# ecmwf-ifs/ecwam

Hardware: AMD Instinct MI355X
Metric: grid-point spectral steps/sec (whole node) at O320, 36dir x 36freq (higher is better)
Workload: dtype f32; 1 GPU; O320 all-ocean octahedral grid, 421080 sea points, 36 dir x 36 freq (NFRE_RED=36), full WAMINTGR step = PROPAGS2 advection + NEWWIND + IMPLSCH as one kernel (PROPAGS2 inside IMPLSCH's tile load), IDELT=IDELPRO=450 s, flag set A (IPHYS=1, ISNONLIN=0, LLGCBZ0=F, LLNORMAGAM=F); points_per_gpu=421080, halo_points=0, parallelism=sea-point block x1, ranks=1

## Files before the change

### ecwam_amd/build.py

```python
from __future__ import annotations

import hashlib
import os
import re
import shutil
import subprocess
import sys

HERE = os.path.dirname(os.path.abspath(__file__))
CSRC = os.path.join(HERE, "csrc")
LIBDIR = os.path.join(HERE, "lib")
LIB = os.path.join(LIBDIR, "libecwam_hip.so")
SOURCES = ["capi.hip", "propag.hip", "implsch4.hip", "implsch4a.hip", "implsch4x.hip", "implsch4r.hip", "implsch4rd.hip", "outbs.hip", "outbs_sep.hip", "outbs_ext.hip"]
DERIVED = {"implsch4r.hip": ("implsch4r.hip", ["-DV4R_PREC=1"]), "implsch4rd.hip": ("implsch4r.hip", ["-DV4R_PREC=2", "-DV4R_DP=2"])}
HIPCC = shutil.which("hipcc") or "/opt/rocm/bin/hipcc"
FAST_DIV = ["-fno-hip-fp32-correctly-rounded-divide-sqrt"]
FLAGS = ["--offload-arch=gfx950", "-O3", "-fPIC", "-std=c++17", "-Wall", "-Wno-unused-variable", "-Wno-unused-but-set-variable"]
IMPLSCH_SOURCES = ("implsch4.hip", "implsch4a.hip", "implsch4x.hip", "implsch4r.hip", "implsch4rd.hip")
VARIANTS = {"": FAST_DIV, "exactdiv": ["-DECWAM_HIP_STRICT=0"], "strict1": ["-DECWAM_HIP_STRICT=1"], "strict2": FAST_DIV + ["-DECWAM_HIP_STRICT=2"],
            "site4": ["-DECWAM_HIP_STRICT=4"], "site8": ["-DECWAM_HIP_STRICT=8"], "site32": ["-DECWAM_HIP_STRICT=32"],
            "strict3": ["-DECWAM_HIP_STRICT=3"], "strict7": ["-DECWAM_HIP_STRICT=3", "-ffp-contract=off"],
            "noieee": FAST_DIV + ["-mno-amdgpu-ieee", "-fno-honor-nans"],
            "rdp": FAST_DIV + ["-O3", "-DV4R_DP=1"], "rdpchk": FAST_DIV + ["-O3", "-DV4R_DP=1", "-DV4_CHECK=1"], "rdpO2": FAST_DIV + ["-O2", "-DV4R_DP=1"],
            "split": FAST_DIV + ["-DV4_SPLIT_ALL=1", "-DV4R_DP=2"],
            "norecpf": FAST_DIV + ["-DV4_RECPF=0"], "norecs": FAST_DIV + ["-DV4_RECV=0"], "noredn": FAST_DIV + ["-DV4_REDN=0"],
            "advprobe": FAST_DIV + ["-DV4_ADV_PROBE=1"],
            "ctustrict": FAST_DIV,
            "advO1": FAST_DIV + ["-O1"],
            "advd2": FAST_DIV + ["-DV4_ADV_DEPTH=2"], "advd4": FAST_DIV + ["-DV4_ADV_DEPTH=4"], "advprio": FAST_DIV + ["-DV4_ADV_PRIO=2"]}
VARIANT_ANY = {"ctustrict": ["-DECWAM_HIP_CTU_STRICT=1"]}
VARIANT_SOURCES = {"ctustrict": ("propag.hip", "implsch4a.hip"), "advprobe": ("implsch4a.hip",), "advO1": ("implsch4a.hip",), "advd2": ("implsch4a.hip",), "advd4": ("implsch4a.hip",),
                   "advprio": ("implsch4a.hip",), "rdp": ("implsch4rd.hip",), "rdpchk": ("implsch4rd.hip",), "rdpO2": ("implsch4rd.hip",),
                   "split": ("implsch4.hip", "implsch4x.hip", "implsch4r.hip", "implsch4rd.hip"), "norecpf": ("implsch4.hip",), "norecs": ("implsch4.hip",),
                   "noredn": ("implsch4.hip",)}

INCLUDE = os.path.join(HERE, "..", "include", "ecwam_hip.h")


def lib_path(variant: str = "") -> str:
    return LIB if not variant else os.path.join(LIBDIR, f"libecwam_hip_{variant}.so")


def _closure(path: str, seen: dict) -> None:
    path = os.path.normpath(path)
    if path in seen or not os.path.exists(path):
        return
    with open(path, "rb") as fh:
        data = fh.read()
    seen[path] = data
    for m in re.finditer(rb'^[ \t]*#[ \t]*include[ \t]*"([^"]+)"', data, re.M):
        _closure(os.path.join(os.path.dirname(path), m.group(1).decode()), seen)


def _stamp(src: str, flags: list) -> str:
    seen: dict = {}
    _closure(os.path.join(CSRC, src), seen)
    h = hashlib.sha256(" ".join([HIPCC, *flags]).encode())
    for k in sorted(seen):
        h.update(os.path.relpath(k, HERE).encode())
        h.update(seen[k])
    return h.hexdigest()


def build(force: bool = False, verbose: bool = False, variant: str = "") -> str:
    if variant not in VARIANTS:
# ... 90 lines not shown
```

### ecwam_amd/csrc/capi.hip

```cpp
#include <cmath>
#include <cstdio>
#include <cstdlib>
#include <cstring>
#include <string>
#include <vector>

#include <dlfcn.h>
#include <rccl/rccl.h>

#include "dev.h"
#include "implsch_adv_args.h"

static thread_local std::string g_err;
static int fail(const std::string& m) {
  g_err = m;
  return 1;
}
#define HIPCHK(x)                                                                        \
  do {                                                                                   \
    hipError_t e_ = (x);                                                                 \
    if (e_ != hipSuccess) return fail(std::string(#x) + ": " + hipGetErrorString(e_));   \
  } while (0)

struct ecwam_hip_ctx {
// ... 736 lines not shown
  if (!c) return fail("null context");
  if (!fused_ok(c) || !implsch4_adv_forms(c->NANG, c->real_bytes)) return fail("ecwam_hip_propags2_implsch: no one-kernel build covers the configuration (ecwam_hip_propags2_implsch_supported): call ecwam_hip_propags2_otf and ecwam_hip_implsch");
  if (kijl < kijs || kijs < 0 || kijl > n || nd3s < 1 || nd3e > c->NFRE_RED || nd3e < nd3s - 1) return fail("ecwam_hip_propags2_implsch: bad range");
  if (kijl > kijs && (!f1 || !f3 || !kxlt || !zdello || !cosph || !sinph || !klon || !klat || !kcor || !wlat || !wcor || !cgroup_ext || !cosphm1_ext ||
                      !wvprpt || !ff || !intf || !mij || !xllws))
    return fail("ecwam_hip_propags2_implsch: null pointer");
  if (f1 == f3) return fail("ecwam_hip_propags2_implsch: F1 and F3 must not alias (the neighbours of a point are read while other points are stored)");
  if (((uintptr_t)f1 % 16) != 0 || ((uintptr_t)f3 % 16) != 0) return fail("ecwam_hip_propags2_implsch: the spectra must be 16-byte aligned");
  if (ifrelfmax < 0 || ifrelfmax > c->NFRE_RED || (ifrelfmax > 0) != (gin != nullptr))
    return fail("ecwam_hip_propags2_implsch: fast waves (ifrelfmax > 0) come with their compact input rows (gin), and only then");
  if (gin && (nd3s != 1 || gin_nfre < ifrelfmax || gin_nfre > c->NFRE || gin_nfre % (16 / c->real_bytes) != 0 || ((uintptr_t)gin % 16) != 0 || gin == c->fast_g ||
              !(delpro_lf > 0.0)))
    return fail("ecwam_hip_propags2_implsch: the compact fast-wave rows must be 16-byte aligned, hold the fast waves in a multiple of 16 bytes per direction, and differ from the rows of ecwam_hip_set_fastwave_copy");
  if (c->p.lwnemocou && kijl > kijs && !wam2nemo) return fail("ecwam_hip_propags2_implsch: LWNEMOCOU needs the WAVE2OCEAN buffer");
  if (c->obs && kijl > c->n_obs) return fail("ecwam_hip_propags2_implsch: more points than the obstruction table holds");
  if (!c->p.lwnemocou) wam2nemo = nullptr;
  HIPCHK(hipSetDevice(c->device));
  hipStream_t s = (hipStream_t)stream;
  if (kijl == kijs) return 0;
  if (int rc2 = implsch_reserve_on(c, kijl, s, false)) return rc2;
  const size_t dir_reals = (size_t)(6 * c->NANG + 4);
  int* dirI = reinterpret_cast<int*>(reinterpret_cast<char*>(c->adv_dir) + dir_reals * c->real_bytes);
  const double dlf = gin ? delpro_lf : 0.0;
  DISPATCH(launch_ctu_prep<float>(c->dtab, kijs, kijl, ngy, delpro, dlf, kxlt, zdello, xdella, cosph, sinph, wlat, wcor, cosphm1_ext, c->adv_pt, c->adv_dir, dirI, s),
           launch_ctu_prep<double>(c->dtab, kijs, kijl, ngy, delpro, dlf, kxlt, zdello, xdella, cosph, sinph, wlat, wcor, cosphm1_ext, c->adv_pt, c->adv_dir, dirI, s));
  Implsch4AdvArgs a;
  a.f_in = f1; a.klon = klon; a.klat = klat; a.kcor = kcor; a.cg = cgroup_ext; a.pt = c->adv_pt; a.dirT = c->adv_dir; a.dirI = dirI;
  a.xdella = xdella; a.delpro = delpro; a.m0 = nd3s - 1; a.m1 = nd3e;
  a.gin = gin; a.delpro_lf = dlf; a.gin_k = gin ? gin_nfre : 0; a.mlf = gin ? ifrelfmax : 0;
  a.obs = c->obs;
  a.gfast = c->fast_g; a.gfast_k = c->fast_g ? c->fast_gk : 0;
  a.xcd_walk = (flags & 1) ? 1 : (((flags >> 8) & 0xFFF) > 1 ? ((flags >> 8) & 0xFFF) : 0);
  a.mode = (flags & 2) ? 2 : 1;
  const int ext = (c->p.llnormagam || c->p.llgcbz0) ? 1 : 0;
  int rc = -1;
  DISPATCH(rc = launch_implsch4_adv<float>(c->dtab, kijs, kijl, f3, wvprpt, ff, intf, mij, xllws, c->fin, wam2nemo, &a, c->NANG, c->NFRE, c->v4_r1, c->v4_r2, c->v4_nh, ext, s),
           rc = launch_implsch4_adv<double>(c->dtab, kijs, kijl, f3, wvprpt, ff, intf, mij, xllws, c->fin, wam2nemo, &a, c->NANG, c->NFRE, c->v4_r1, c->v4_r2, c->v4_nh, ext, s));
  if (rc != 0) return fail("ecwam_hip_propags2_implsch: no one-kernel build covers the configuration (the strict build of the weights has neither the fast-wave nor the obstruction form)");
  HIPCHK(hipGetLastError());
  c->implsch_last = 4;
  return 0;
}

int ecwam_hip_set_fastwave_copy(ecwam_hip_ctx* c, void* g, int g_nfre) {
  if (!c) return fail("null context");
  if (g && (g_nfre < 1 || g_nfre > c->NFRE || g_nfre % (16 / c->real_bytes) != 0 || ((uintptr_t)g % 16) != 0))
    return fail("ecwam_hip_set_fastwave_copy: the compact rows must be 16-byte aligned and hold a multiple of 16 bytes per direction");
  c->fast_g = g; c->fast_gk = g ? g_nfre : 0;
  return 0;
}

static int implsch_reserve_on(ecwam_hip_ctx* c, int npts, hipStream_t s, bool sync) {
  HIPCHK(hipSetDevice(c->device));
  const size_t need = (size_t)(npts > 0 ? npts : 0) * implsch4_fin_row() * c->real_bytes;
  if (need > c->fin_bytes) {
    if (c->fin) HIPCHK(hipFree(c->fin));
    c->fin = nullptr; c->fin_bytes = 0;
    HIPCHK(hipMalloc(&c->fin, need));
    HIPCHK(hipMemsetAsync(c->fin, 0, need, s));
    HIPCHK(hipStreamSynchronize(s));
    (void)sync;
    c->fin_bytes = need;
  }
  const bool split = implsch4_split_all() || (c->real_bytes == 8 && implsch4r_dp_split() && runs_rare_builds(c));
  const size_t need_wi = split ? (size_t)(npts > 0 ? npts : 0) * c->NANG * c->NFRE * c->real_bytes : 0;
  if (need_wi > c->wi_bytes) {
// ... 429 lines not shown
```

### ecwam_amd/csrc/implsch4a.hip

```cpp
#include "implsch_v4_launch.h"
#include "implsch_adv_args.h"

#ifndef V4_ADV_PROBE
#define V4_ADV_PROBE 0
#endif

template <typename T>
int launch_implsch4_adv(const void* tab, int kijs, int kijl, void* fl_out, const void* wvprpt, void* ff, void* intf, int* mij, void* xllws, void* fin,
                        double* w2n, const Implsch4AdvArgs* a, int NANG, int NFRE, int r1, int r2, int nh, int ext, hipStream_t s) {
  if (kijl - kijs <= 0) return 0;
  if (NFRE != V4_NFRE) return -1;
  V4Adv<T> adv;
  adv.f_in = (const T*)a->f_in; adv.klon = a->klon; adv.klat = a->klat; adv.kcor = a->kcor; adv.cg = (const T*)a->cg; adv.pt = (const T*)a->pt;
  adv.dirT = (const T*)a->dirT; adv.dirI = a->dirI; adv.xdella = (T)a->xdella; adv.delpro = (T)a->delpro; adv.m0 = a->m0; adv.m1 = a->m1;
  adv.xcd_walk = a->xcd_walk;
  adv.gin = (const T*)a->gin; adv.delpro_lf = (T)a->delpro_lf; adv.gin_k = a->gin_k; adv.mlf = a->mlf; adv.obs = (const T*)a->obs;
#define V4_ARGS tab, kijs, kijl, fl_out, wvprpt, ff, intf, mij, xllws, fin, w2n, a->gfast, a->gfast_k, adv, s
#define V4_ADV_CASE(NA, PPV, R1V, R2V, NHV, LFOK)                                                                                         \
  if (NANG == NA && r1 == R1V && r2 == R2V && nh == NHV) {                                                                              \
    if (a->mode != 1) return -1;                                                                                                        \
    const int form = (a->gin ? 2 : 0) | (a->obs ? 4 : 0);                                                                               \
    if (!a->gin && a->mlf != 0) return -1;                                                                                              \
    if (form == 0) return ext ? launch4_adv<T, NA, PPV, R1V, R2V, NHV, true, 1>(V4_ARGS) : launch4_adv<T, NA, PPV, R1V, R2V, NHV, false, 1>(V4_ARGS); \
    if constexpr (!ECWAM_HIP_CTU_STRICT) {       \
      if (form == 4) return ext ? launch4_adv<T, NA, PPV, R1V, R2V, NHV, true, 5>(V4_ARGS) : launch4_adv<T, NA, PPV, R1V, R2V, NHV, false, 5>(V4_ARGS); \
      if constexpr (LFOK) {                                                                                                             \
        if (form == 2) return ext ? launch4_adv<T, NA, PPV, R1V, R2V, NHV, true, 3>(V4_ARGS) : launch4_adv<T, NA, PPV, R1V, R2V, NHV, false, 3>(V4_ARGS); \
        if (form == 6) return ext ? launch4_adv<T, NA, PPV, R1V, R2V, NHV, true, 7>(V4_ARGS) : launch4_adv<T, NA, PPV, R1V, R2V, NHV, false, 7>(V4_ARGS); \
      }                                                                                                                                 \
    }                                                                                                                                   \
    return -1;                                                                                                                          \
  }
  constexpr bool SP = sizeof(T) == 4;
#if V4_ADV_PROBE
  if constexpr (SP)
    if (NANG == 36 && r1 == 1 && r2 == 3 && nh == 8 && a->mode == 2) return ext ? -1 : launch4_adv<T, 36, 3, 1, 3, 8, false, 2>(V4_ARGS);
#endif
  V4_ADV_CASE(36, (SP ? 3 : V4_DP36_PP), 1, 3, 8, true)
  if constexpr (SP) {
    V4_ADV_CASE(24, 5, 0, 2, 5, true)
    V4_ADV_CASE(12, 10, 0, 1, 3, true)
    V4_ADV_CASE(48, 2, 1, 4, 11, false)
  }
#undef V4_ADV_CASE
#undef V4_ARGS
  return -1;
}
template int launch_implsch4_adv<float>(const void*, int, int, void*, const void*, void*, void*, int*, void*, void*, double*, const Implsch4AdvArgs*, int, int, int, int, int, int, hipStream_t);
// ... 7 lines not shown
```

### ecwam_amd/csrc/implsch_adv_args.h

```cpp
#pragma once
struct Implsch4AdvArgs {
  const void* f_in;
  const int *klon, *klat, *kcor;
  const void* cg;
  const void* pt;
  const void* dirT;
  const int* dirI;
  double xdella, delpro;
  const void* gin;
  double delpro_lf;
  int gin_k, mlf;
  const void* obs;
  void* gfast;
  int gfast_k;
  int m0, m1;
  int xcd_walk;
  int mode;
};
```

### ecwam_amd/csrc/implsch_v4.h

```cpp
#pragma once
#include "ctu.h"

#define V4_NFRE 36
#ifdef ECWAM_HIP_DIAGNOSTICS
#define V4_PHASE_EXIT(k) do { if (tb.DBG_SKIP == (k)) return; } while (0)
#else
#define V4_PHASE_EXIT(k) do { } while (0)
#endif
#if defined(V4_CHECK) && V4_CHECK
#include <cassert>
#define V4_CHK(c) assert(c)
#else
#define V4_CHK(c) do { } while (0)
#endif
#define V4_NSTG 4
#define V4_NS(nang) ((V4_NFRE + (nang) / 2 - 1) / ((nang) / 2))
#define V4_PLN(pp, nang) ((pp) * ((nang) > V4_NFRE ? (nang) : V4_NFRE))
#define V4_NFAC 6

#define V4SYNC() WSYNC()
#define V4_WPE_MIN(T) (sizeof(T) == 4 ? 2 : 1)

template <typename T>
using V2 = T __attribute__((ext_vector_type(2)));

enum { FIN_AIRD = 0, FIN_UFRIC, FIN_Z0M, FIN_MIJ, FIN_XS, FIN_YS, FIN_F1DCOS3, FIN_F1DCOS2, FIN_F1DSIN2, FIN_F1D, FIN_RNFAC, FIN_PHIWA,
       FIN_SINWD, FIN_COSWD, FIN_WSWAVE, FIN_CICOVER, FIN_PHILF, FIN_XSTRESS, FIN_YSTRESS, FIN_Z0B, FIN_CHRNCK, FIN_COSDIFF, FIN_EMEAN, FIN_F1MEAN,
       FIN_TAUICX, FIN_TAUICY, FIN_STRNMS, FIN_SPARE,
       FIN_FMEAN, FIN_FMEANWS, FIN_AKMEAN, FIN_XKMEAN, FIN_SDS, FIN_SC, V4_NFIN = 36 };

__device__ __forceinline__ float v4_bp(int addr, float v) { return __int_as_float(__builtin_amdgcn_ds_bpermute(addr, __float_as_int(v))); }
__device__ __forceinline__ double v4_bp(int addr, double v) {
  const int lo = __builtin_amdgcn_ds_bpermute(addr, __double2loint(v));
  const int hi = __builtin_amdgcn_ds_bpermute(addr, __double2hiint(v));
// ... 221 lines not shown

template <typename T, int NANG_, int PP_>
struct V4Ctx {
  int lane, p, j;
  T* tile;
  int own;
  T* fac4;
  T* sq;
  T* zcn;
  T* c;
  V4Rot<T> rot;
  V2<T> sinth, costh;
  T rDFIM, rDFIMOFR, rDFIMFR, rZPIFR, rRHOWG, rCOFRM4, rFLMAX;
};
enum { Q4_BSC = 0, Q4_SBO, Q4_CINV, Q4_WAVNUM };

template <typename T>
struct V4Adv {
  const T* f_in;
  const int* klon;
  const int* klat;
  const int* kcor;
  const T* cg;
  const T* pt;
  const T* dirT;
  const int* dirI;
  T xdella, delpro;
  const T* gin;
  T delpro_lf;
  int gin_k, mlf;
  const T* obs;
  int m0, m1;
  int xcd_walk;
};
#ifndef V4_ADV_DEPTH
#define V4_ADV_DEPTH 3
#endif
template <typename T, int NANG, int PP, int MODE, int NSCR>
__device__ __forceinline__ void v4_advect_tile(const V4Adv<T>& A, int ij0, int n, int lane, T* __restrict__ sT, T* __restrict__ sScr) {
  constexpr int NFRE = V4_NFRE, N = NANG * NFRE, RS = PP * NANG, VEC = 16 / (int)sizeof(T), NC = NFRE / VEC, NVL = N / VEC;
  constexpr int NFULL = NVL / 64, NREM = NVL - 64 * NFULL, NTS = (PP * NREM + 63) / 64, NCH = NFULL * PP + NTS, D = V4_ADV_DEPTH;
  constexpr int PTW = 20;
  typedef T VT __attribute__((ext_vector_type(VEC)));
  typedef int I4 __attribute__((ext_vector_type(4)));
  T* sB = sScr;
  T* sPt = sB + PP * 5 * NFRE;
  T* sK = sPt + PP * PTW;
  constexpr bool LF = (MODE & 3) == 3;
  constexpr bool OBS = (MODE & 4) != 0;
  constexpr int NB = OBS ? 11 : 8;
  static_assert(MODE == 2 || (MODE & 1), "modes: 1 plain, 3 fast waves, + 4 obstructions; 2 the probe");
  constexpr int NKW = NANG * 4 + 4 + (LF ? NANG * 2 : 0);
  int* sI = reinterpret_cast<int*>(sK + NKW);
  int* sD = sI + PP * 16;
  static_assert((PP * 5 * NFRE + PP * PTW + NKW) * sizeof(T) + (PP * 16 + NANG * 4) * sizeof(int) <= NSCR * sizeof(T), "LDS scratch of the advecting load");
  for (int i = lane; i < PP * PTW; i += 64) {
    const int q = i / PTW, e = i - q * PTW;
    const T* g = A.pt + (size_t)(ij0 + (q < n ? q : n - 1)) * 12;
    T v = T(0);
    if (e < 12) v = g[e];
    else if (e < 18) v = T(1) - g[e - 6];
    else if (e == 18) v = g[0] * g[2];
    else v = A.xdella * g[2];
    if (e == 1) v = m_abs(v);
    sPt[i] = v;
  }
  for (int i = lane; i < PP * 16; i += 64) {
    const int q = i >> 4, e = i & 15;
    const int ijq = ij0 + (q < n ? q : n - 1);
    int v = ijq;
    if (e >= 1 && e <= 2) v = A.klon[(size_t)ijq * 2 + (e - 1)];
    if (e >= 3 && e <= 6) v = A.klat[(size_t)ijq * 4 + (e - 3)];
    if (e >= 7 && e <= 14) v = A.kcor[(size_t)ijq * 8 + (e - 7)];
    sI[i] = v;
  }
  for (int i = lane; i < NKW; i += 64) {
    const T v = A.dirT[i];
    const int e = i & 3;
    sK[i] = i >= NANG * 4 + 4 ? T(2) * v : (i >= NANG * 4 ? v : (e < 2 ? T(2) * v : m_abs(v)));
  }
  for (int i = lane; i < NANG * 4; i += 64) sD[i] = A.dirI[i];
  WSYNC();
#if defined(V4_ADV_PRIO)
  __builtin_amdgcn_s_setprio(V4_ADV_PRIO);
#endif
  VT buf[D][NB];
  auto chunk_of = [&](int c, int& q, int& k, int& m) {
    int w;
    if (c < NFULL * PP) {
      const int it = c / PP;
      q = c - it * PP;
      w = lane + 64 * it;
    } else {
      int t = lane + 64 * (c - NFULL * PP);
      t = t < PP * NREM ? t : PP * NREM - 1;
      q = t / (NREM > 0 ? NREM : 1);
      w = 64 * NFULL + (t - q * NREM);
    }
    k = w / NC;
    m = (w - k * NC) * VEC;
  };
  auto issue = [&](int c, VT (&b)[NB]) {
    int q, k, m;
    chunk_of(c, q, k, m);
    const I4 dk = *reinterpret_cast<const I4*>(sD + 4 * k);
    const int jx0 = dk.x & 1, jy0 = (dk.x >> 1) & 1, kc = (dk.x >> 2) & 3;
    const int* iq = sI + q * 16;
    const bool fromg = LF && m < A.gin_k;
    const T* src = fromg ? A.gin : A.f_in;
    const int rk = fromg ? A.gin_k : NFRE;
    const size_t rn = (size_t)NANG * rk;
    const T* own = src + (size_t)iq[0] * rn;
    const int el = k * rk + m;
    b[0] = *reinterpret_cast<const VT*>(own + el);
    b[1] = *reinterpret_cast<const VT*>(src + (size_t)iq[1 + jx0] * rn + el);
    b[2] = *reinterpret_cast<const VT*>(src + (size_t)iq[3 + 2 * jy0] * rn + el);
    b[3] = *reinterpret_cast<const VT*>(src + (size_t)iq[4 + 2 * jy0] * rn + el);
    b[4] = *reinterpret_cast<const VT*>(src + (size_t)iq[7 + 2 * kc] * rn + el);
    b[5] = *reinterpret_cast<const VT*>(src + (size_t)iq[8 + 2 * kc] * rn + el);
    b[6] = *reinterpret_cast<const VT*>(own + dk.y * rk + m);
    b[7] = *reinterpret_cast<const VT*>(own + dk.z * rk + m);
    if constexpr (OBS) {
      const T* o = A.obs + (size_t)iq[0] * 8 * NFRE + m;
      b[8] = *reinterpret_cast<const VT*>(o + (2 + jx0) * NFRE);
      b[9] = *reinterpret_cast<const VT*>(o + jy0 * NFRE);
      b[10] = *reinterpret_cast<const VT*>(o + (4 + kc) * NFRE);
    }
  };
  auto finish = [&](int c, const VT (&b)[NB]) {
    int q, k, m;
    chunk_of(c, q, k, m);
    T r[VEC];
    if constexpr (MODE == 2) {
#pragma unroll
      for (int i = 0; i < VEC; i++) r[i] = T(0.3) * b[0][i] + T(0.1) * (((b[1][i] + b[2][i]) + (b[3][i] + b[4][i])) + ((b[5][i] + b[6][i]) + b[7][i]));
    } else {
      const int sel = sD[4 * k];
      const int jx0 = sel & 1, jy0 = (sel >> 1) & 1, kc = (sel >> 2) & 3;
      const T* pq = sPt + q * PTW;
      const T zd = pq[0], acpm1 = pq[1], ga = pq[2], tanph = pq[3], wl = pq[6 + jy0], omwl = pq[12 + jy0], wc = pq[8 + kc], omwc = pq[14 + kc];
      const T cmtodeg = sK[NANG * 4];
      const VT kk = *reinterpret_cast<const VT*>(sK + 4 * k);
      const T kk2 = sizeof(T) == 4 ? kk[2 % VEC] : sK[4 * k + 2], kk3 = sizeof(T) == 4 ? kk[3 % VEC] : sK[4 * k + 3];
#if ECWAM_HIP_CTU_STRICT
      T a2, b2, p2, m2;
      {
#pragma clang fp contract(off)
        const T tsp2 = tanph * kk[0], tsm2 = tanph * kk[1];
        a2 = m_max(tsp2, T(0)); p2 = m_max(-tsp2, T(0)); b2 = m_max(-tsm2, T(0)); m2 = m_max(tsm2, T(0));
      }
#else
      T ab2, p2, m2;
      ctu_fast_dir<T>(tanph, kk[0], kk[1], ab2, p2, m2);
      T ab2_lf = ab2, p2_lf = p2, m2_lf = m2;
      if constexpr (LF) ctu_fast_dir<T>(tanph, sK[NANG * 4 + 4 + 2 * k], sK[NANG * 4 + 4 + 2 * k + 1], ab2_lf, p2_lf, m2_lf);
#endif
      const T* bb = sB + q * 5 * NFRE + m;
      const VT bha = *reinterpret_cast<const VT*>(bb + jx0 * NFRE), bhb = *reinterpret_cast<const VT*>(bb + (1 - jx0) * NFRE),
               bya = *reinterpret_cast<const VT*>(bb + (2 + jy0) * NFRE), byb = *reinterpret_cast<const VT*>(bb + (3 - jy0) * NFRE),
               bc0 = *reinterpret_cast<const VT*>(bb + 4 * NFRE);
#if ECWAM_HIP_CTU_STRICT
      static_assert(!LF && !OBS, "the strict build of the weights has the plain form only");
#pragma unroll
      for (int i = 0; i < VEC; i += 2) {
#define P2(a) V2<T>{a[i], a[i + 1]}
        const V2<T> rr = ctu_w8_stencil_abs<T>(P2(bha), P2(bhb), P2(bya), P2(byb), P2(bc0), kk2, kk3, acpm1, zd, A.xdella, ga, A.delpro, cmtodeg, wl, omwl,
                                               wc, omwc, a2, b2, p2, m2, P2(b[0]), P2(b[1]), P2(b[2]), P2(b[3]), P2(b[4]), P2(b[5]), P2(b[6]), P2(b[7]));
#undef P2
        r[i] = rr.x; r[i + 1] = rr.y;
      }
#else
      const T zdg = pq[18], xdg = pq[19];
#pragma unroll
      for (int i = 0; i < VEC; i += 2) {
#define P2(a) V2<T>{a[i], a[i + 1]}
        const bool lf0 = LF && (m + i) < A.mlf, lf1 = LF && (m + i + 1) < A.mlf;
        CtuFastW8<T> w = ctu_fast_w8<T>(P2(bha), P2(bhb), P2(bya), P2(byb), P2(bc0), kk2, kk3, zd, A.xdella, ga, zdg, xdg, wl, omwl, wc, omwc,
                                        V2<T>{lf0 ? ab2_lf : ab2, lf1 ? ab2_lf : ab2}, V2<T>{lf0 ? p2_lf : p2, lf1 ? p2_lf : p2},
                                        V2<T>{lf0 ? m2_lf : m2, lf1 ? m2_lf : m2});
        if constexpr (OBS) {
          w.wlon = w.wlon * P2(b[8]); w.wlat1 = w.wlat1 * P2(b[9]); w.wlat2 = w.wlat2 * P2(b[9]); w.wcor1 = w.wcor1 * P2(b[10]); w.wcor2 = w.wcor2 * P2(b[10]);
        }
        const V2<T> rr = ctu_fast_apply<T>(w, P2(b[0]), P2(b[1]), P2(b[2]), P2(b[3]), P2(b[4]), P2(b[5]), P2(b[6]), P2(b[7]));
#undef P2
        r[i] = rr.x; r[i + 1] = rr.y;
      }
#endif
#pragma unroll
      for (int i = 0; i < VEC; i++)
        if (m + i < A.m0 || m + i >= A.m1) r[i] = b[0][i];
    }
    T* d = sT + m * RS + q * NANG + k;
#pragma unroll
    for (int i = 0; i < VEC; i++) d[i * RS] = r[i];
  };
#pragma unroll
  for (int c = 0; c < D - 1 && c < NCH; c++) issue(c, buf[c % D]);
  __builtin_amdgcn_sched_barrier(0);
  if constexpr ((MODE & 1) != 0) {
    for (int i = lane; i < PP * NFRE; i += 64) {
      const int q = i / NFRE, m = i - q * NFRE;
      const int* iq = sI + q * 16;
      const T* pq = sPt + q * PTW;
      T cgl[2], cgy0[2], cgy1[2];
#pragma unroll
      for (int ic = 0; ic < 2; ic++) {
        cgl[ic] = A.cg[(size_t)iq[1 + ic] * NFRE + m];
        cgy0[ic] = A.cg[(size_t)iq[3 + 2 * ic] * NFRE + m];
        cgy1[ic] = A.cg[(size_t)iq[4 + 2 * ic] * NFRE + m];
      }
      const T wl[2] = {pq[6], pq[7]}, dp[2] = {pq[4], pq[5]};
      const CtuBase<T> b = ctu_base(A.cg[(size_t)iq[0] * NFRE + m], cgl, cgy0, cgy1, wl, dp);
      T* o = sB + q * 5 * NFRE + m;
#if ECWAM_HIP_CTU_STRICT
      o[0] = m_abs(b.h[0]); o[NFRE] = m_abs(b.h[1]); o[2 * NFRE] = m_abs(b.hy[0]); o[3 * NFRE] = m_abs(b.hy[1]); o[4 * NFRE] = b.cg0;
#else
      ctu_fast_planes<T>(b, pq[1], ((LF && m < A.mlf) ? A.delpro_lf : A.delpro) * sK[NANG * 4], o, o + NFRE, o + 2 * NFRE, o + 3 * NFRE);
      o[4 * NFRE] = b.cg0;
#endif
    }
    WSYNC();
  }
#pragma unroll
  for (int c = 0; c < NCH; c++) {
    if (c + D - 1 < NCH) issue(c + D - 1, buf[(c + D - 1) % D]);
    __builtin_amdgcn_sched_barrier(0);
    finish(c, buf[c % D]);
    __builtin_amdgcn_sched_barrier(0);
  }
#if defined(V4_ADV_PRIO)
  __builtin_amdgcn_s_setprio(0);
#endif
  WSYNC();
}

template <typename T>
__device__ T stress_gc_row(const DevTab<T>& tb, int l16, bool run, T ANG_GC, T USTAR, T Z0, T Z0MIN, T HALP, T RNFAC) {
  const T XLAMA = T(0.25), XLAMB = T(4.0);
  const int NS = ns_gc_d(tb, USTAR);
  const T t = USTAR * (Z0MIN / Z0);
  const T TAUWCG_MIN = t * t;
  const T XLAMBDA = T(1) + XLAMA * m_tanh(XLAMB * m_pow4(USTAR));
  const T LOGXL = m_log(XLAMBDA);
  const T hc = HALP * tb.C2OSQRTVG_GC[NS];
  const T ZABHRC = ANG_GC * tb.BETAMAXOXKAPPA2 * hc;
  const T CONST = tb.LLNORMAGAM ? RNFAC * tb.BMAXOKAP * hc / m_max(USTAR, tb.EPSUS) : T(0);
  T acc = T(0);
  for (int I = NS + l16;; I += 16) {
    const bool act = run && I <= tb.NWAV_GC;
    if (__builtin_amdgcn_ballot_w64(act) == 0ull) break;
    if (act) {
      const T X = USTAR * tb.CM_GC[I];
      const T XLOG = m_log(tb.XK_GC[I] * Z0) + tb.XKAPPA / (X + tb.ZALP);
      const T ZLOG = m_min(XLOG - LOGXL, T(0));
      const T ZLOG2X = ZLOG * ZLOG * X;
      const T GAM_W = ZLOG2X * ZLOG2X * m_exp(XLOG) * tb.OM3GMKM_GC[I];
      const T ZN = CONST * tb.XKMSQRTVGOC2_GC[I] * GAM_W;
      const T GAMNORMA = (T(1) + tb.RN1_RN * ZN) / (T(1) + ZN);
      const T wt = (I == NS) ? tb.DELKCC_GC_NS[NS] * tb.OMXKM3_GC[NS] : tb.DELKCC_OMXKM3_GC[I];
      acc = acc + (GAM_W * wt) * GAMNORMA;
    }
  }
  const T TAUWCG = v4_rowsum<T>(V2<T>{acc, T(0)}).x;
  return m_max(ZABHRC * TAUWCG, TAUWCG_MIN);
}
// ... 1751 lines not shown
```

Before: 59.62 million grid-point spectral steps/s.

## Use 32-bit gather offsets from a shared base in the advecting tile load

Each block computes the min and max neighbour index with a wave reduction. When the gathered rows fit within 4 GiB of a common base, it precomputes per-neighbour 32-bit byte offsets in LDS and issues global loads as base plus unsigned offset, avoiding 64-bit address arithmetic for each of the eight to eleven stencil loads. The direction table is packed into two ints to shrink LDS reads, and a specialisation drops the carry-through branch when the full frequency range is advected. It also removes the depth and priority build variants, and it adds LDS use plus a third instantiation of the load loop, which grows code size.

After: 60.14 million grid-point spectral steps/s, median of 6. No clear change (+0.9%).

```diff
diff --git a/ecwam_amd/build.py b/ecwam_amd/build.py
--- a/ecwam_amd/build.py
+++ b/ecwam_amd/build.py
@@ -26,11 +26,9 @@
             "norecpf": FAST_DIV + ["-DV4_RECPF=0"], "norecs": FAST_DIV + ["-DV4_RECV=0"], "noredn": FAST_DIV + ["-DV4_REDN=0"],
             "advprobe": FAST_DIV + ["-DV4_ADV_PROBE=1"],
             "ctustrict": FAST_DIV,
-            "advO1": FAST_DIV + ["-O1"],
-            "advd2": FAST_DIV + ["-DV4_ADV_DEPTH=2"], "advd4": FAST_DIV + ["-DV4_ADV_DEPTH=4"], "advprio": FAST_DIV + ["-DV4_ADV_PRIO=2"]}
+            "advO1": FAST_DIV + ["-O1"]}
 VARIANT_ANY = {"ctustrict": ["-DECWAM_HIP_CTU_STRICT=1"]}
-VARIANT_SOURCES = {"ctustrict": ("propag.hip", "implsch4a.hip"), "advprobe": ("implsch4a.hip",), "advO1": ("implsch4a.hip",), "advd2": ("implsch4a.hip",), "advd4": ("implsch4a.hip",),
-                   "advprio": ("implsch4a.hip",), "rdp": ("implsch4rd.hip",), "rdpchk": ("implsch4rd.hip",), "rdpO2": ("implsch4rd.hip",),
+VARIANT_SOURCES = {"ctustrict": ("propag.hip", "implsch4a.hip"), "advprobe": ("implsch4a.hip",), "advO1": ("implsch4a.hip",), "rdp": ("implsch4rd.hip",), "rdpchk": ("implsch4rd.hip",), "rdpO2": ("implsch4rd.hip",),
                    "split": ("implsch4.hip", "implsch4x.hip", "implsch4r.hip", "implsch4rd.hip"), "norecpf": ("implsch4.hip",), "norecs": ("implsch4.hip",),
                    "noredn": ("implsch4.hip",)}
 
diff --git a/ecwam_amd/csrc/capi.hip b/ecwam_amd/csrc/capi.hip
--- a/ecwam_amd/csrc/capi.hip
+++ b/ecwam_amd/csrc/capi.hip
@@ -792,6 +792,7 @@
   a.gfast = c->fast_g; a.gfast_k = c->fast_g ? c->fast_gk : 0;
   a.xcd_walk = (flags & 1) ? 1 : (((flags >> 8) & 0xFFF) > 1 ? ((flags >> 8) & 0xFFF) : 0);
   a.mode = (flags & 2) ? 2 : 1;
+  a.gather64 = (flags & 4) ? 1 : 0;
   const int ext = (c->p.llnormagam || c->p.llgcbz0) ? 1 : 0;
   int rc = -1;
   DISPATCH(rc = launch_implsch4_adv<float>(c->dtab, kijs, kijl, f3, wvprpt, ff, intf, mij, xllws, c->fin, wam2nemo, &a, c->NANG, c->NFRE, c->v4_r1, c->v4_r2, c->v4_nh, ext, s),
diff --git a/ecwam_amd/csrc/implsch4a.hip b/ecwam_amd/csrc/implsch4a.hip
--- a/ecwam_amd/csrc/implsch4a.hip
+++ b/ecwam_amd/csrc/implsch4a.hip
@@ -13,7 +13,7 @@
   V4Adv<T> adv;
   adv.f_in = (const T*)a->f_in; adv.klon = a->klon; adv.klat = a->klat; adv.kcor = a->kcor; adv.cg = (const T*)a->cg; adv.pt = (const T*)a->pt;
   adv.dirT = (const T*)a->dirT; adv.dirI = a->dirI; adv.xdella = (T)a->xdella; adv.delpro = (T)a->delpro; adv.m0 = a->m0; adv.m1 = a->m1;
-  adv.xcd_walk = a->xcd_walk;
+  adv.xcd_walk = a->xcd_walk; adv.gather64 = a->gather64;
   adv.gin = (const T*)a->gin; adv.delpro_lf = (T)a->delpro_lf; adv.gin_k = a->gin_k; adv.mlf = a->mlf; adv.obs = (const T*)a->obs;
 #define V4_ARGS tab, kijs, kijl, fl_out, wvprpt, ff, intf, mij, xllws, fin, w2n, a->gfast, a->gfast_k, adv, s
 #define V4_ADV_CASE(NA, PPV, R1V, R2V, NHV, LFOK)                                                                                         \
diff --git a/ecwam_amd/csrc/implsch_adv_args.h b/ecwam_amd/csrc/implsch_adv_args.h
--- a/ecwam_amd/csrc/implsch_adv_args.h
+++ b/ecwam_amd/csrc/implsch_adv_args.h
@@ -15,5 +15,6 @@
   int gfast_k;
   int m0, m1;
   int xcd_walk;
+  int gather64;
   int mode;
 };
diff --git a/ecwam_amd/csrc/implsch_v4.h b/ecwam_amd/csrc/implsch_v4.h
--- a/ecwam_amd/csrc/implsch_v4.h
+++ b/ecwam_amd/csrc/implsch_v4.h
@@ -1,5 +1,6 @@
 #pragma once
 #include "ctu.h"
+#include <type_traits>
 
 #define V4_NFRE 36
 #ifdef ECWAM_HIP_DIAGNOSTICS
@@ -287,6 +288,7 @@
   const T* obs;
   int m0, m1;
   int xcd_walk;
+  int gather64;
 };
 #ifndef V4_ADV_DEPTH
 #define V4_ADV_DEPTH 3
@@ -297,7 +299,7 @@
   constexpr int NFULL = NVL / 64, NREM = NVL - 64 * NFULL, NTS = (PP * NREM + 63) / 64, NCH = NFULL * PP + NTS, D = V4_ADV_DEPTH;
   constexpr int PTW = 20;
   typedef T VT __attribute__((ext_vector_type(VEC)));
-  typedef int I4 __attribute__((ext_vector_type(4)));
+  typedef int I2 __attribute__((ext_vector_type(2)));
   T* sB = sScr;
   T* sPt = sB + PP * 5 * NFRE;
   T* sK = sPt + PP * PTW;
@@ -306,9 +308,12 @@
   constexpr int NB = OBS ? 11 : 8;
   static_assert(MODE == 2 || (MODE & 1), "modes: 1 plain, 3 fast waves, + 4 obstructions; 2 the probe");
   constexpr int NKW = NANG * 4 + 4 + (LF ? NANG * 2 : 0);
+  constexpr int NSO = LF ? 2 : 1;
   int* sI = reinterpret_cast<int*>(sK + NKW);
-  int* sD = sI + PP * 16;
-  static_assert((PP * 5 * NFRE + PP * PTW + NKW) * sizeof(T) + (PP * 16 + NANG * 4) * sizeof(int) <= NSCR * sizeof(T), "LDS scratch of the advecting load");
+  unsigned* sO = reinterpret_cast<unsigned*>(sI + PP * 16);
+  int* sD = reinterpret_cast<int*>(sO + NSO * PP * 16);
+  static_assert((PP * 5 * NFRE + PP * PTW + NKW) * sizeof(T) + (PP * 16 * (1 + NSO) + NANG * 2) * sizeof(int) <= NSCR * sizeof(T),
+                "LDS scratch of the advecting load");
   for (int i = lane; i < PP * PTW; i += 64) {
     const int q = i / PTW, e = i - q * PTW;
     const T* g = A.pt + (size_t)(ij0 + (q < n ? q : n - 1)) * 12;
@@ -320,6 +325,7 @@
     if (e == 1) v = m_abs(v);
     sPt[i] = v;
   }
+  int lo = 0x7FFFFFFF, hi = 0;
   for (int i = lane; i < PP * 16; i += 64) {
     const int q = i >> 4, e = i & 15;
     const int ijq = ij0 + (q < n ? q : n - 1);
@@ -328,164 +334,215 @@
     if (e >= 3 && e <= 6) v = A.klat[(size_t)ijq * 4 + (e - 3)];
     if (e >= 7 && e <= 14) v = A.kcor[(size_t)ijq * 8 + (e - 7)];
     sI[i] = v;
+    lo = v < lo ? v : lo;
+    hi = v > hi ? v : hi;
+  }
+#pragma unroll
+  for (int o = 32; o > 0; o >>= 1) {
+    const int lo2 = __shfl_xor(lo, o), hi2 = __shfl_xor(hi, o);
+    lo = lo2 < lo ? lo2 : lo;
+    hi = hi2 > hi ? hi2 : hi;
+  }
+  lo = __builtin_amdgcn_readfirstlane(lo);
+  hi = __builtin_amdgcn_readfirstlane(hi);
+  const uint64_t rbf = (uint64_t)NANG * NFRE * sizeof(T), rbg = LF ? (uint64_t)NANG * (uint64_t)A.gin_k * sizeof(T) : 0;
+  const uint64_t pf = (uint64_t)(uintptr_t)A.f_in + (uint64_t)lo * rbf, pg = LF ? (uint64_t)(uintptr_t)A.gin + (uint64_t)lo * rbg : pf;
+  const uint64_t pb = pg < pf ? pg : pf, span = (uint64_t)(hi - lo + 1);
+  const bool fast = !A.gather64 && (pf - pb) + span * rbf <= (1ull << 32) && (!LF || (pg - pb) + span * rbg <= (1ull << 32));
+  typedef const __attribute__((address_space(1))) char* GP;
+  const GP base = reinterpret_cast<GP>((uintptr_t)pb);
+  for (int i = lane; i < PP * 16; i += 64) {
+    const uint64_t d = (uint64_t)(sI[i] - lo);
+    sO[i] = (unsigned)((pf - pb) + d * rbf);
+    if constexpr (LF) sO[PP * 16 + i] = (unsigned)((pg - pb) + d * rbg);
   }
   for (int i = lane; i < NKW; i += 64) {
     const T v = A.dirT[i];
     const int e = i & 3;
     sK[i] = i >= NANG * 4 + 4 ? T(2) * v : (i >= NANG * 4 ? v : (e < 2 ? T(2) * v : m_abs(v)));
   }
-  for (int i = lane; i < NANG * 4; i += 64) sD[i] = A.dirI[i];
+  for (int i = lane; i < NANG * 2; i += 64) sD[i] = (i & 1) ? A.dirI[2 * i - 1] | A.dirI[2 * i] << 16 : A.dirI[2 * i];
   WSYNC();
-#if defined(V4_ADV_PRIO)
-  __builtin_amdgcn_s_setprio(V4_ADV_PRIO);
-#endif
-  VT buf[D][NB];
-  auto chunk_of = [&](int c, int& q, int& k, int& m) {
-    int w;
+  const GP obase = reinterpret_cast<GP>(OBS ? (uintptr_t)(A.obs + (size_t)ij0 * 8 * NFRE) : (uintptr_t)0);
+  const int k0 = lane / NC, r0 = lane - k0 * NC;
+  auto chunk_of = [&](int c, int& q, int& k, int& m, int& w) {
     if (c < NFULL * PP) {
       const int it = c / PP;
       q = c - it * PP;
       w = lane + 64 * it;
+      const int a = 64 * it / NC, b = 64 * it - a * NC, r = r0 + b;
+      const bool cy = r >= NC;
+      k = k0 + a + (cy ? 1 : 0);
+      m = (cy ? r - NC : r) * VEC;
     } else {
       int t = lane + 64 * (c - NFULL * PP);
       t = t < PP * NREM ? t : PP * NREM - 1;
       q = t / (NREM > 0 ? NREM : 1);
       w = 64 * NFULL + (t - q * NREM);
-    }
-    k = w / NC;
-    m = (w - k * NC) * VEC;
+      k = w / NC;
+      m = (w - k * NC) * VEC;
+    }
   };
-  auto issue = [&](int c, VT (&b)[NB]) {
-    int q, k, m;
-    chunk_of(c, q, k, m);
-    const I4 dk = *reinterpret_cast<const I4*>(sD + 4 * k);
-    const int jx0 = dk.x & 1, jy0 = (dk.x >> 1) & 1, kc = (dk.x >> 2) & 3;
-    const int* iq = sI + q * 16;
-    const bool fromg = LF && m < A.gin_k;
-    const T* src = fromg ? A.gin : A.f_in;
-    const int rk = fromg ? A.gin_k : NFRE;
-    const size_t rn = (size_t)NANG * rk;
-    const T* own = src + (size_t)iq[0] * rn;
-    const int el = k * rk + m;
-    b[0] = *reinterpret_cast<const VT*>(own + el);
-    b[1] = *reinterpret_cast<const VT*>(src + (size_t)iq[1 + jx0] * rn + el);
-    b[2] = *reinterpret_cast<const VT*>(src + (size_t)iq[3 + 2 * jy0] * rn + el);
-    b[3] = *reinterpret_cast<const VT*>(src + (size_t)iq[4 + 2 * jy0] * rn + el);
-    b[4] = *reinterpret_cast<const VT*>(src + (size_t)iq[7 + 2 * kc] * rn + el);
-    b[5] = *reinterpret_cast<const VT*>(src + (size_t)iq[8 + 2 * kc] * rn + el);
-    b[6] = *reinterpret_cast<const VT*>(own + dk.y * rk + m);
-    b[7] = *reinterpret_cast<const VT*>(own + dk.z * rk + m);
-    if constexpr (OBS) {
-      const T* o = A.obs + (size_t)iq[0] * 8 * NFRE + m;
-      b[8] = *reinterpret_cast<const VT*>(o + (2 + jx0) * NFRE);
-      b[9] = *reinterpret_cast<const VT*>(o + jy0 * NFRE);
-      b[10] = *reinterpret_cast<const VT*>(o + (4 + kc) * NFRE);
+  auto run = [&](auto fast_c, auto carry_c) {
+    constexpr bool FAST = decltype(fast_c)::value, CARRY = decltype(carry_c)::value;
+    VT buf[D][NB];
+    auto issue = [&](int c, VT (&b)[NB]) {
+      int q, k, m, w;
+      chunk_of(c, q, k, m, w);
+      const I2 dk = *reinterpret_cast<const I2*>(sD + 2 * k);
+      const int jx0 = dk.x & 1, jy0 = (dk.x >> 1) & 1, kc = (dk.x >> 2) & 3, km = dk.y & 0xFFFF, kp = dk.y >> 16;
+      const bool fromg = LF && m < A.gin_k;
+      const int rk = fromg ? A.gin_k : NFRE;
+      if constexpr (FAST) {
+        const unsigned* oq = sO + (fromg ? PP * 16 : 0) + q * 16;
+        const unsigned el = fromg ? (unsigned)(k * rk + m) * (unsigned)sizeof(T) : (unsigned)w * 16u;
+        auto ld = [&](unsigned off) { return *reinterpret_cast<const __attribute__((address_space(1))) VT*>(base + off); };
+        const unsigned o0 = oq[0];
+        b[0] = ld(o0 + el);
+        b[1] = ld(oq[1 + jx0] + el);
+        b[2] = ld(oq[3 + 2 * jy0] + el);
+        b[3] = ld(oq[4 + 2 * jy0] + el);
+        b[4] = ld(oq[7 + 2 * kc] + el);
+        b[5] = ld(oq[8 + 2 * kc] + el);
+        b[6] = ld(o0 + (unsigned)(km * rk + m) * (unsigned)sizeof(T));
+        b[7] = ld(o0 + (unsigned)(kp * rk + m) * (unsigned)sizeof(T));
+        if constexpr (OBS) {
+          const unsigned o = (unsigned)(((q < n ? q : n - 1) * 8 * NFRE + m) * (int)sizeof(T));
+          auto ldo = [&](int j) { return *reinterpret_cast<const __attribute__((address_space(1))) VT*>(obase + o + (unsigned)(j * NFRE * (int)sizeof(T))); };
+          b[8] = ldo(2 + jx0);
+          b[9] = ldo(jy0);
+          b[10] = ldo(4 + kc);
+        }
+      } else {
+        const int* iq = sI + q * 16;
+        const T* src = fromg ? A.gin : A.f_in;
+        const size_t rn = (size_t)NANG * rk;
+        const T* own = src + (size_t)iq[0] * rn;
+        const int el = k * rk + m;
+        b[0] = *reinterpret_cast<const VT*>(own + el);
+        b[1] = *reinterpret_cast<const VT*>(src + (size_t)iq[1 + jx0] * rn + el);
+        b[2] = *reinterpret_cast<const VT*>(src + (size_t)iq[3 + 2 * jy0] * rn + el);
+        b[3] = *reinterpret_cast<const VT*>(src + (size_t)iq[4 + 2 * jy0] * rn + el);
+        b[4] = *reinterpret_cast<const VT*>(src + (size_t)iq[7 + 2 * kc] * rn + el);
+        b[5] = *reinterpret_cast<const VT*>(src + (size_t)iq[8 + 2 * kc] * rn + el);
+        b[6] = *reinterpret_cast<const VT*>(own + km * rk + m);
+        b[7] = *reinterpret_cast<const VT*>(own + kp * rk + m);
+        if constexpr (OBS) {
+          const T* o = A.obs + (size_t)iq[0] * 8 * NFRE + m;
+          b[8] = *reinterpret_cast<const VT*>(o + (2 + jx0) * NFRE);
+          b[9] = *reinterpret_cast<const VT*>(o + jy0 * NFRE);
+          b[10] = *reinterpret_cast<const VT*>(o + (4 + kc) * NFRE);
+        }
+      }
+    };
+    auto finish = [&](int c, const VT (&b)[NB]) {
+      int q, k, m, wch;
+      chunk_of(c, q, k, m, wch);
+      T r[VEC];
+      if constexpr (MODE == 2) {
+#pragma unroll
+        for (int i = 0; i < VEC; i++) r[i] = T(0.3) * b[0][i] + T(0.1) * (((b[1][i] + b[2][i]) + (b[3][i] + b[4][i])) + ((b[5][i] + b[6][i]) + b[7][i]));
+      } else {
+        const int sel = sD[2 * k];
+        const int jx0 = sel & 1, jy0 = (sel >> 1) & 1, kc = (sel >> 2) & 3;
+        const T* pq = sPt + q * PTW;
+        const T zd = pq[0], acpm1 = pq[1], ga = pq[2], tanph = pq[3], wl = pq[6 + jy0], omwl = pq[12 + jy0], wc = pq[8 + kc], omwc = pq[14 + kc];
+        const T cmtodeg = sK[NANG * 4];
+        const VT kk = *reinterpret_cast<const VT*>(sK + 4 * k);
+        const T kk2 = sizeof(T) == 4 ? kk[2 % VEC] : sK[4 * k + 2], kk3 = sizeof(T) == 4 ? kk[3 % VEC] : sK[4 * k + 3];
+#if ECWAM_HIP_CTU_STRICT
+        T a2, b2, p2, m2;
+        {
+#pragma clang fp contract(off)
+          const T tsp2 = tanph * kk[0], tsm2 = tanph * kk[1];
+          a2 = m_max(tsp2, T(0)); p2 = m_max(-tsp2, T(0)); b2 = m_max(-tsm2, T(0)); m2 = m_max(tsm2, T(0));
+        }
+#else
+        T ab2, p2, m2;
+        ctu_fast_dir<T>(tanph, kk[0], kk[1], ab2, p2, m2);
+        T ab2_lf = ab2, p2_lf = p2, m2_lf = m2;
+        if constexpr (LF) ctu_fast_dir<T>(tanph, sK[NANG * 4 + 4 + 2 * k], sK[NANG * 4 + 4 + 2 * k + 1], ab2_lf, p2_lf, m2_lf);
+#endif
+        const T* bb = sB + q * 5 * NFRE + m;
+        const VT bha = *reinterpret_cast<const VT*>(bb + jx0 * NFRE), bhb = *reinterpret_cast<const VT*>(bb + (1 - jx0) * NFRE),
+                 bya = *reinterpret_cast<const VT*>(bb + (2 + jy0) * NFRE), byb = *reinterpret_cast<const VT*>(bb + (3 - jy0) * NFRE),
+                 bc0 = *reinterpret_cast<const VT*>(bb + 4 * NFRE);
+#if ECWAM_HIP_CTU_STRICT
+        static_assert(!LF && !OBS, "the strict build of the weights has the plain form only");
+#pragma unroll
+        for (int i = 0; i < VEC; i += 2) {
+#define P2(a) V2<T>{a[i], a[i + 1]}
+          const V2<T> rr = ctu_w8_stencil_abs<T>(P2(bha), P2(bhb), P2(bya), P2(byb), P2(bc0), kk2, kk3, acpm1, zd, A.xdella, ga, A.delpro, cmtodeg, wl, omwl,
+                                                 wc, omwc, a2, b2, p2, m2, P2(b[0]), P2(b[1]), P2(b[2]), P2(b[3]), P2(b[4]), P2(b[5]), P2(b[6]), P2(b[7]));
+#undef P2
+          r[i] = rr.x; r[i + 1] = rr.y;
+        }
+#else
+        const T zdg = pq[18], xdg = pq[19];
+#pragma unroll
+        for (int i = 0; i < VEC; i += 2) {
+#define P2(a) V2<T>{a[i], a[i + 1]}
+          const bool lf0 = LF && (m + i) < A.mlf, lf1 = LF && (m + i + 1) < A.mlf;
+          CtuFastW8<T> w = ctu_fast_w8<T>(P2(bha), P2(bhb), P2(bya), P2(byb), P2(bc0), kk2, kk3, zd, A.xdella, ga, zdg, xdg, wl, omwl, wc, omwc,
+                                          V2<T>{lf0 ? ab2_lf : ab2, lf1 ? ab2_lf : ab2}, V2<T>{lf0 ? p2_lf : p2, lf1 ? p2_lf : p2},
+                                          V2<T>{lf0 ? m2_lf : m2, lf1 ? m2_lf : m2});
+          if constexpr (OBS) {
+            w.wlon = w.wlon * P2(b[8]); w.wlat1 = w.wlat1 * P2(b[9]); w.wlat2 = w.wlat2 * P2(b[9]); w.wcor1 = w.wcor1 * P2(b[10]); w.wcor2 = w.wcor2 * P2(b[10]);
+          }
+          const V2<T> rr = ctu_fast_apply<T>(w, P2(b[0]), P2(b[1]), P2(b[2]), P2(b[3]), P2(b[4]), P2(b[5]), P2(b[6]), P2(b[7]));
+#undef P2
+          r[i] = rr.x; r[i + 1] = rr.y;
+        }
+#endif
+        if constexpr (CARRY) {
+#pragma unroll
+          for (int i = 0; i < VEC; i++)
+            if (m + i < A.m0 || m + i >= A.m1) r[i] = b[0][i];
+        }
+      }
+      T* d = sT + m * RS + q * NANG + k;
+#pragma unroll
+      for (int i = 0; i < VEC; i++) d[i * RS] = r[i];
+    };
+#pragma unroll
+    for (int c = 0; c < D - 1 && c < NCH; c++) issue(c, buf[c % D]);
+    __builtin_amdgcn_sched_barrier(0);
+    if constexpr ((MODE & 1) != 0) {
+      for (int i = lane; i < PP * NFRE; i += 64) {
+        const int q = i / NFRE, m = i - q * NFRE;
+        const int* iq = sI + q * 16;
+        const T* pq = sPt + q * PTW;
+        T cgl[2], cgy0[2], cgy1[2];
+#pragma unroll
+        for (int ic = 0; ic < 2; ic++) {
+          cgl[ic] = A.cg[(size_t)iq[1 + ic] * NFRE + m];
+          cgy0[ic] = A.cg[(size_t)iq[3 + 2 * ic] * NFRE + m];
+          cgy1[ic] = A.cg[(size_t)iq[4 + 2 * ic] * NFRE + m];
+        }
+        const T wl[2] = {pq[6], pq[7]}, dp[2] = {pq[4], pq[5]};
+        const CtuBase<T> b = ctu_base(A.cg[(size_t)iq[0] * NFRE + m], cgl, cgy0, cgy1, wl, dp);
+        T* o = sB + q * 5 * NFRE + m;
+#if ECWAM_HIP_CTU_STRICT
+        o[0] = m_abs(b.h[0]); o[NFRE] = m_abs(b.h[1]); o[2 * NFRE] = m_abs(b.hy[0]); o[3 * NFRE] = m_abs(b.hy[1]); o[4 * NFRE] = b.cg0;
+#else
+        ctu_fast_planes<T>(b, pq[1], ((LF && m < A.mlf) ? A.delpro_lf : A.delpro) * sK[NANG * 4], o, o + NFRE, o + 2 * NFRE, o + 3 * NFRE);
+        o[4 * NFRE] = b.cg0;
+#endif
+      }
+      WSYNC();
+    }
+#pragma unroll
+    for (int c = 0; c < NCH; c++) {
+      if (c + D - 1 < NCH) issue(c + D - 1, buf[(c + D - 1) % D]);
+      __builtin_amdgcn_sched_barrier(0);
+      finish(c, buf[c % D]);
+      __builtin_amdgcn_sched_barrier(0);
     }
   };
-  auto finish = [&](int c, const VT (&b)[NB]) {
-    int q, k, m;
-    chunk_of(c, q, k, m);
-    T r[VEC];
-    if constexpr (MODE == 2) {
-#pragma unroll
-      for (int i = 0; i < VEC; i++) r[i] = T(0.3) * b[0][i] + T(0.1) * (((b[1][i] + b[2][i]) + (b[3][i] + b[4][i])) + ((b[5][i] + b[6][i]) + b[7][i]));
-    } else {
-      const int sel = sD[4 * k];
-      const int jx0 = sel & 1, jy0 = (sel >> 1) & 1, kc = (sel >> 2) & 3;
-      const T* pq = sPt + q * PTW;
-      const T zd = pq[0], acpm1 = pq[1], ga = pq[2], tanph = pq[3], wl = pq[6 + jy0], omwl = pq[12 + jy0], wc = pq[8 + kc], omwc = pq[14 + kc];
-      const T cmtodeg = sK[NANG * 4];
-      const VT kk = *reinterpret_cast<const VT*>(sK + 4 * k);
-      const T kk2 = sizeof(T) == 4 ? kk[2 % VEC] : sK[4 * k + 2], kk3 = sizeof(T) == 4 ? kk[3 % VEC] : sK[4 * k + 3];
-#if ECWAM_HIP_CTU_STRICT
-      T a2, b2, p2, m2;
-      {
-#pragma clang fp contract(off)
-        const T tsp2 = tanph * kk[0], tsm2 = tanph * kk[1];
-        a2 = m_max(tsp2, T(0)); p2 = m_max(-tsp2, T(0)); b2 = m_max(-tsm2, T(0)); m2 = m_max(tsm2, T(0));
-      }
-#else
-      T ab2, p2, m2;
-      ctu_fast_dir<T>(tanph, kk[0], kk[1], ab2, p2, m2);
-      T ab2_lf = ab2, p2_lf = p2, m2_lf = m2;
-      if constexpr (LF) ctu_fast_dir<T>(tanph, sK[NANG * 4 + 4 + 2 * k], sK[NANG * 4 + 4 + 2 * k + 1], ab2_lf, p2_lf, m2_lf);
-#endif
-      const T* bb = sB + q * 5 * NFRE + m;
-      const VT bha = *reinterpret_cast<const VT*>(bb + jx0 * NFRE), bhb = *reinterpret_cast<const VT*>(bb + (1 - jx0) * NFRE),
-               bya = *reinterpret_cast<const VT*>(bb + (2 + jy0) * NFRE), byb = *reinterpret_cast<const VT*>(bb + (3 - jy0) * NFRE),
-               bc0 = *reinterpret_cast<const VT*>(bb + 4 * NFRE);
-#if ECWAM_HIP_CTU_STRICT
-      static_assert(!LF && !OBS, "the strict build of the weights has the plain form only");
-#pragma unroll
-      for (int i = 0; i < VEC; i += 2) {
-#define P2(a) V2<T>{a[i], a[i + 1]}
-        const V2<T> rr = ctu_w8_stencil_abs<T>(P2(bha), P2(bhb), P2(bya), P2(byb), P2(bc0), kk2, kk3, acpm1, zd, A.xdella, ga, A.delpro, cmtodeg, wl, omwl,
-                                               wc, omwc, a2, b2, p2, m2, P2(b[0]), P2(b[1]), P2(b[2]), P2(b[3]), P2(b[4]), P2(b[5]), P2(b[6]), P2(b[7]));
-#undef P2
-        r[i] = rr.x; r[i + 1] = rr.y;
-      }
-#else
-      const T zdg = pq[18], xdg = pq[19];
-#pragma unroll
-      for (int i = 0; i < VEC; i += 2) {
-#define P2(a) V2<T>{a[i], a[i + 1]}
-        const bool lf0 = LF && (m + i) < A.mlf, lf1 = LF && (m + i + 1) < A.mlf;
-        CtuFastW8<T> w = ctu_fast_w8<T>(P2(bha), P2(bhb), P2(bya), P2(byb), P2(bc0), kk2, kk3, zd, A.xdella, ga, zdg, xdg, wl, omwl, wc, omwc,
-                                        V2<T>{lf0 ? ab2_lf : ab2, lf1 ? ab2_lf : ab2}, V2<T>{lf0 ? p2_lf : p2, lf1 ? p2_lf : p2},
-                                        V2<T>{lf0 ? m2_lf : m2, lf1 ? m2_lf : m2});
-        if constexpr (OBS) {
-          w.wlon = w.wlon * P2(b[8]); w.wlat1 = w.wlat1 * P2(b[9]); w.wlat2 = w.wlat2 * P2(b[9]); w.wcor1 = w.wcor1 * P2(b[10]); w.wcor2 = w.wcor2 * P2(b[10]);
-        }
-        const V2<T> rr = ctu_fast_apply<T>(w, P2(b[0]), P2(b[1]), P2(b[2]), P2(b[3]), P2(b[4]), P2(b[5]), P2(b[6]), P2(b[7]));
-#undef P2
-        r[i] = rr.x; r[i + 1] = rr.y;
-      }
-#endif
-#pragma unroll
-      for (int i = 0; i < VEC; i++)
-        if (m + i < A.m0 || m + i >= A.m1) r[i] = b[0][i];
-    }
-    T* d = sT + m * RS + q * NANG + k;
-#pragma unroll
-    for (int i = 0; i < VEC; i++) d[i * RS] = r[i];
-  };
-#pragma unroll
-  for (int c = 0; c < D - 1 && c < NCH; c++) issue(c, buf[c % D]);
-  __builtin_amdgcn_sched_barrier(0);
-  if constexpr ((MODE & 1) != 0) {
-    for (int i = lane; i < PP * NFRE; i += 64) {
-      const int q = i / NFRE, m = i - q * NFRE;
-      const int* iq = sI + q * 16;
-      const T* pq = sPt + q * PTW;
-      T cgl[2], cgy0[2], cgy1[2];
-#pragma unroll
-      for (int ic = 0; ic < 2; ic++) {
-        cgl[ic] = A.cg[(size_t)iq[1 + ic] * NFRE + m];
-        cgy0[ic] = A.cg[(size_t)iq[3 + 2 * ic] * NFRE + m];
-        cgy1[ic] = A.cg[(size_t)iq[4 + 2 * ic] * NFRE + m];
-      }
-      const T wl[2] = {pq[6], pq[7]}, dp[2] = {pq[4], pq[5]};
-      const CtuBase<T> b = ctu_base(A.cg[(size_t)iq[0] * NFRE + m], cgl, cgy0, cgy1, wl, dp);
-      T* o = sB + q * 5 * NFRE + m;
-#if ECWAM_HIP_CTU_STRICT
-      o[0] = m_abs(b.h[0]); o[NFRE] = m_abs(b.h[1]); o[2 * NFRE] = m_abs(b.hy[0]); o[3 * NFRE] = m_abs(b.hy[1]); o[4 * NFRE] = b.cg0;
-#else
-      ctu_fast_planes<T>(b, pq[1], ((LF && m < A.mlf) ? A.delpro_lf : A.delpro) * sK[NANG * 4], o, o + NFRE, o + 2 * NFRE, o + 3 * NFRE);
-      o[4 * NFRE] = b.cg0;
-#endif
-    }
-    WSYNC();
-  }
-#pragma unroll
-  for (int c = 0; c < NCH; c++) {
-    if (c + D - 1 < NCH) issue(c + D - 1, buf[(c + D - 1) % D]);
-    __builtin_amdgcn_sched_barrier(0);
-    finish(c, buf[c % D]);
-    __builtin_amdgcn_sched_barrier(0);
-  }
-#if defined(V4_ADV_PRIO)
-  __builtin_amdgcn_s_setprio(0);
-#endif
+  const bool all_m = A.m0 == 0 && A.m1 == NFRE;
+  if (fast && all_m) run(std::true_type{}, std::false_type{});
+  else if (fast) run(std::true_type{}, std::true_type{});
+  else run(std::false_type{}, std::true_type{});
   WSYNC();
 }
 
```
